# chpio/crdt-enc

Measured on AMD Instinct MI355X. Metric: op files compacted/sec + AEAD-open GB/s, 1M×4KiB ops/4096 actors, 1–8 GPUs, higher is better.
Workload: dtype u32; 1 GPU; C2: 1,048,576 x 4 KiB encrypted GCounter op files per GPU (4096 actors x 256 versions at N=1), decrypt + max-join + compact; plaintext_bytes=4085, actors=4096, parallelism=single GPU

## Files before the change

crdt-enc_amd/crdtenc.py:

```python
import ctypes
import os

HERE = os.path.dirname(os.path.abspath(__file__))
LIB_PATH = os.environ.get("CRDTENC_LIB") or os.path.join(HERE, "libcrdtenc.so")

OK = 0
STATUS_NAMES = {
    0: "OK", 1: "OUTER_LEN", 2: "OUTER_VERSION", 3: "KEY_VERSION", 4: "KEY_LEN",
    5: "PARSE_VBOX", 6: "DATA_VERSION", 7: "PARSE_ENCBOX", 8: "NONCE_LEN", 9: "AUTH",
    10: "PT_LEN", 11: "PT_VERSION", 12: "DECODE", 13: "OP_VERSION", 64: "INVALID_ARG",
    65: "DEVICE", 66: "NO_KEY", 67: "IO", 68: "NO_LOCAL_META", 69: "SHARD",
}
ERR_OP_VERSION, ERR_SHARD = 13, 69
SHARD_BAD, SHARD_GAP, SHARD_E0_MISMATCH = 1, 2, 4
STATE_VCLOCK, STATE_GCOUNTER, STATE_ORSWOT, STATE_MVREG, STATE_PNCOUNTER = 0, 1, 2, 3, 4
STATE_GSET = 5
OPEN_CREATE, COMPACT_INGEST_FORMAT, OPEN_MULTI_KEY = 1, 2, 4

CORE_VERSION = bytes.fromhex("e834d789101b463498239de990a9051f")
KEY_VERSION = bytes.fromhex("5df28591439a4cef8ca68433276cc9ed")

EXPORTS = [
    "ce_buf_free", "ce_status_str", "ce_ctx_create", "ce_ctx_destroy", "ce_ctx_set_stream",
    "ce_ctx_synchronize", "ce_ctx_last_error", "ce_cryptor_gen_key", "ce_cryptor_encrypt",
    "ce_cryptor_decrypt", "ce_cryptor_sealed_len", "ce_cryptor_decrypt_batch",
    "ce_cryptor_encrypt_batch", "ce_cryptor_decrypt_batch_device",
    "ce_cryptor_encrypt_batch_device", "ce_storage_open", "ce_storage_close",
    "ce_storage_list_op_actors", "ce_storage_load_ops", "ce_storage_store_ops",
    "ce_storage_remove_ops", "ce_storage_list_state_names", "ce_storage_store_state",
    "ce_storage_load_state", "ce_storage_remove_state", "ce_content_name", "ce_content_name_async",
    "ce_content_name_wait", "ce_core_open",
    "ce_core_close", "ce_core_set_latest_key", "ce_core_info_actor", "ce_core_read_remote",
    "ce_core_compact", "ce_core_apply_ops", "ce_core_state_bytes", "ce_core_ingest_ops",
    "ce_core_ingest_ops_device", "ce_core_ingest_states", "ce_core_compact_to_buffer",
    "ce_core_compact_into", "ce_core_compact_ops_device",
    "ce_core_register_actors", "ce_core_dense_capacity", "ce_core_export_dense",
    "ce_core_import_dense", "ce_vbuf_init", "ce_vbuf_remaining", "ce_vbuf_chunk",
    "ce_vbuf_advance", "ce_vbuf_chunks_vectored", "ce_ctx_set_timing", "ce_ctx_timing_read",
    "ce_ctx_timing_reset", "ce_ctx_set_timing_only", "ce_core_reset", "ce_core_settle", "ce_core_merge_state", "ce_core_dense_ready",
    "ce_keys_decode", "ce_keys_from_remote_metas", "ce_keys_merge", "ce_keys_free",
    "ce_keys_count", "ce_keys_latest", "ce_keys_get", "ce_keys_at", "ce_core_set_keys",
    "ce_core_apply_ops_batch", "ce_core_ingest_ops_iov", "ce_core_ingest_states_iov", "ce_core_compact_ops_iov",
    "ce_core_path_count", "ce_ctx_clock_probe",
    "ce_shard_owner", "ce_shard_owners", "ce_shard_stats_len", "ce_core_shard_stats",
    "ce_core_shard_window", "ce_core_ingest_ops_device_sharded", "ce_core_pending_export",
    "ce_core_pending_commit", "ce_core_writer_versions", "ce_shard_stats_host",
    "ce_shard_window_host", "ce_shard_window_exact", "ce_core_compact_ops_device_into",
    "ce_core_state_bytes_device", "ce_core_merge_state_device", "ce_core_export_columns_device",
    "ce_core_merge_columns_device", "ce_core_ingest_states_device",
    "ce_core_compact_into_async", "ce_core_compact_wait", "ce_host_alloc", "ce_host_free", "ce_content_names",
    "ce_core_gset_ingest_ops_device_sharded", "ce_core_gset_pending_members", "ce_core_gset_pending_commit",
    "ce_core_set_contains_device", "ce_core_set_contains", "ce_core_set_len", "ce_core_set_members_device",
    "ce_core_counter_read", "ce_core_clock_get", "ce_core_read_clock", "ce_core_orswot_member_clocks",
    "ce_core_mvreg_read",
]


class _HostMem:

    def __init__(self, n):
        self.p = lib().ce_host_alloc(n)
        if not self.p:
            raise MemoryError("ce_host_alloc(%d)" % n)

    def __del__(self):
        try:
# ... 285 lines not shown

    def set_timing(self, enable=True):
        self.check(lib().ce_ctx_set_timing(self.p, 1 if enable else 0), "set_timing")

    def set_timing_only(self, kernel=None):
        self.check(lib().ce_ctx_set_timing_only(self.p, kernel.encode() if kernel else None),
                   "set_timing_only")

    def timing(self, kernel):
        ms = ctypes.c_double(0)
        cnt = ctypes.c_uint64(0)
        self.check(lib().ce_ctx_timing_read(self.p, kernel.encode(), ctypes.byref(ms),
                                            ctypes.byref(cnt)), "timing")
        return ms.value, cnt.value

    def timing_reset(self):
        lib().ce_ctx_timing_reset(self.p)

    def clock_probe(self, out_ptr, blocks, samples, ticks, stream_ptr=None):
        self.check(lib().ce_ctx_clock_probe(self.p, ctypes.c_void_p(stream_ptr), ctypes.c_void_p(out_ptr),
                                            ctypes.c_uint32(blocks), ctypes.c_uint32(samples),
                                            ctypes.c_uint32(ticks)), "clock_probe")

    def gen_key(self):
        b = Buf()
        self.check(lib().ce_cryptor_gen_key(self.p, ctypes.byref(b)), "gen_key")
        vb = _take(b)
        return vb[:16], vb[16:]

    def encrypt(self, key, clear, nonce=None, key_version=KEY_VERSION):
        b = Buf()
        rc = lib().ce_cryptor_encrypt(self.p, _cbuf(key_version), _cbuf(key),
                                      ctypes.c_size_t(len(key)),
                                      _cbuf(nonce) if nonce is not None else None,
                                      _cbuf(clear), ctypes.c_size_t(len(clear)), ctypes.byref(b))
        self.check(rc, "encrypt")
        return _take(b)

    def decrypt(self, key, enc, key_version=KEY_VERSION):
        b = Buf()
        rc = lib().ce_cryptor_decrypt(self.p, _cbuf(key_version), _cbuf(key),
                                      ctypes.c_size_t(len(key)), _cbuf(enc),
                                      ctypes.c_size_t(len(enc)), ctypes.byref(b))
        if rc:
            return rc, None
        return 0, _take(b)
# ... 599 lines not shown
```

crdt-enc_amd/csrc/ce_core.cpp:

```cpp
#include <algorithm>
#include <atomic>
#include <cstdio>
#include <functional>
#include <set>

#include "ce_core.h"
#include "ce_shard.h"

using namespace ce;

namespace ce {


bool skip_any(Rd& r, int depth) {
  if (depth > 1024) return false;
  uint64_t at, cnt = 0;
  if (r.i >= r.n) return false;
  const uint8_t m = r.p[r.i];
  bool cont = false;
  if ((m & 0xf0) == 0x80) { r.i++; cnt = 2ull * (m & 15); cont = true; }
  else if ((m & 0xf0) == 0x90) { r.i++; cnt = m & 15; cont = true; }
  else if (m == 0xdc || m == 0xdd || m == 0xde || m == 0xdf) {
    r.i++;
    if (!rd_be(r, (m == 0xdc || m == 0xde) ? 2 : 4, &cnt)) return false;
// ... 784 lines not shown
    if (rg) return rg;
  }
  DecodeArgs da{};
  da.pt = ctx->out.as<uint8_t>();
  da.blob = d_blob;
  da.params = ctx->params.as<FileParams>();
  da.aux = ctx->poly_aux.as<PolyAux>();
  da.status = ctx->status.as<int32_t>();
  da.n = n;
  da.supported = c->d_supported.as<uint8_t>();
  da.n_supported = (uint32_t)c->supported.size();
  da.apply = ctx->apply.as<uint8_t>();
  da.counters = ctx->counters.as<uint32_t>();
  da.miss_list = ctx->miss.as<uint4>();
  da.miss_cap = 65536;
  da.refold = ctx->refold.as<uint8_t>();
  da.table = c->d_table.as<ActorSlot>();
  da.mask = c->cap - 1;
  da.nil_actor = table_has_nil(c);
  da.batch = c->d_batch.as<unsigned long long>();
  da.large_list = ctx->large.as<uint32_t>();

  ctx->open_log.grid_cap = test_grid_cap();
  auto run_fold = [&](const uint8_t* only) -> int {
    da.only = only;
    da.large_only = 1;
    if (pnc) {
      hipEvent_t t0, t1;
      (void)ctx->tlaunch("open_fold_small", &t0, &t1);
      if ((e = launch_open_fold_pn(ctx->stream, da, ctx->open_log, t0, t1))) return ctx->hip_fail(e, "fused");
    } else if (c->fused == 2 && c->files_per_wave != 1) {
      hipEvent_t t0, t1;
      (void)ctx->tlaunch("open_fold_small", &t0, &t1);
      if ((e = launch_open_fold_v2(ctx->stream, da, c->files_per_wave, ctx->open_log, t0, t1))) return ctx->hip_fail(e, "fused");
    } else {
      const int t = ctx->tbegin("open_fold_small");
      if ((e = launch_open_fold_small(ctx->stream, da, c->files_per_wave, ctx->open_log))) return ctx->hip_fail(e, "fused");
      ctx->tend(t);
    }
    count_open_launches(c, ctx);
    if (!setup_known) {
      if (hsetup_dev) {
        volatile const uint32_t* hp = hsetup;
        for (uint64_t i = 0; hp[16] != gen; i++) {
          if (i >= 64) sched_yield();
          if (i == (1ull << 22)) {
            if ((e = hipStreamSynchronize(ctx->stream))) return ctx->hip_fail(e, "setup counters");
          } else if (i > (1ull << 22) && hp[16] != gen) {
            return ctx->fail(CE_ERR_DEVICE, "setup counters never published");
// ... 1560 lines not shown
```

crdt-enc_amd/csrc/ce_ctx.cpp:

```cpp
#include <sys/random.h>

#include <algorithm>
#include <cstdio>

#include "ce_internal.h"

namespace ce {

hipError_t DevBuf::reserve(size_t bytes) {
  if (bytes <= cap) return hipSuccess;
  if (p) (void)hipFree(p);
  p = nullptr;
  cap = 0;
  size_t want = std::max<size_t>(bytes, 256);
  want = (want + 4095) & ~size_t(4095);
  hipError_t e = hipMalloc(&p, want);
  if (e == hipSuccess) cap = want;
  return e;
}
DevBuf::~DevBuf() {
  if (p) (void)hipFree(p);
}
hipError_t HostBuf::reserve(size_t bytes) {
  if (bytes <= cap) return hipSuccess;
// ... 14 lines not shown
  size_t got = 0;
  while (got < n) {
    ssize_t r = getrandom(out + got, n - got, 0);
    if (r > 0) got += (size_t)r;
  }
}

int32_t key_status(const KeyRef& k) {
  if (std::memcmp(k.version, kKeyVersion, 16) != 0) return CE_ERR_KEY_VERSION;
  if (k.len != 32) return CE_ERR_KEY_LEN;
  return CE_OK;
}

DevKey dev_key(const KeyRef& k) {
  DevKey d{};
  if (k.len == 32) std::memcpy(d.k, k.key, 32);
  return d;
}

uint32_t test_grid_cap() {
  const char* e = getenv("CE_TEST_GRID_CAP");
  const long v = e ? atol(e) : 0;
  return v < 1 ? 0u : (uint32_t)std::min<long>(v, 1l << 30);
}

uint32_t grid_waves_for(uint32_t work) {
  uint32_t full = 256u * 32u;
  if (const uint32_t cap = test_grid_cap()) full = std::min(full, cap);
  return std::max<uint32_t>(1, std::min<uint32_t>(work, full));
}

static int reserve_batch(ce_ctx* ctx, uint32_t n, uint64_t blob_len, uint32_t* extra_cap,
                         uint32_t seg_blocks = kSegBlocks) {
  const uint64_t ec = blob_len / (seg_blocks * 16) + 16;
  if (ec > 0xffffffffull) return ctx->fail(CE_ERR_INVALID_ARG, "batch too large");
  *extra_cap = (uint32_t)ec;
  hipError_t e;
  if ((e = ctx->params.reserve((size_t)n * sizeof(FileParams))) != hipSuccess ||
      (e = ctx->status.reserve((size_t)n * 4 + 64)) != hipSuccess ||
      (e = ctx->counters.reserve(256)) != hipSuccess ||
      (e = ctx->extra.reserve(ec * 8)) != hipSuccess ||
      (e = ctx->multi.reserve(ec * 4)) != hipSuccess ||
      (e = ctx->partials.reserve(ec * 2 * 5 * 4)) != hipSuccess ||
      (e = ctx->large.reserve((size_t)n * 4 + 64)) != hipSuccess ||
      (e = ctx->h_counters.reserve(256)) != hipSuccess)
    return ctx->hip_fail(e, "reserve batch scratch");
// ... 45 lines not shown
}

int device_open(ce_ctx* ctx, const uint8_t* d_blob, const uint64_t* d_offs, uint32_t n,
                uint64_t blob_len, bool outer, const KeyRef& key, uint8_t* d_out,
                int32_t* d_status, bool sync_counters, bool small_lanes, const DecodeArgs* ds) {
  uint32_t ec;
  int rc = reserve_batch(ctx, n, blob_len, &ec);
  if (rc) return rc;
  hipError_t e;
  if ((e = reset_counters(ctx)) != hipSuccess) return ctx->hip_fail(e, "memset counters");
  SegScratch sc = segscratch(ctx, ec);
  FileParams* P = ctx->params.as<FileParams>();
  static const bool ds8_on = !(getenv("CE_DS8") && atoi(getenv("CE_DS8")) == 0);
  const bool want_aux = small_lanes && ds && ds->ds.on && ds->ds.big && ds8_on;
  if (want_aux && (e = ctx->poly_aux.reserve((size_t)n * sizeof(PolyAux))) != hipSuccess)
    return ctx->hip_fail(e, "reserve poly aux");
  int t = ctx->tbegin("open_setup");
  if ((e = launch_open_setup(ctx->stream, d_blob, d_offs, n, outer, dev_key(key), key_status(key),
                             P, d_status, sc, want_aux ? ctx->poly_aux.as<PolyAux>() : nullptr)) != hipSuccess)
    return ctx->hip_fail(e, "open setup");
  ctx->tend(t);
  if (small_lanes) {
    ctx->open_log.grid_cap = test_grid_cap();
    DecodeArgs da{};
    da.pt = d_out;
    da.blob = d_blob;
    da.params = P;
    da.status = d_status;
    da.n = n;
    da.counters = ctx->counters.as<uint32_t>();
    if (ds) {
      da.ds = ds->ds;
      da.aux = want_aux ? ctx->poly_aux.as<PolyAux>() : nullptr;
      da.supported = ds->supported;
      da.n_supported = ds->n_supported;
      da.table = ds->table;
      da.mask = ds->mask;
    }
    t = ctx->tbegin("open_small");
    if ((e = launch_open_small_v2(ctx->stream, da, ctx->open_log)) != hipSuccess) return ctx->hip_fail(e, "open small");
    ctx->tend(t);
  }
  t = ctx->tbegin("segments_open");
  if ((e = launch_segments(ctx->stream, false, d_blob, d_out, P, n, d_status, sc,
                           grid_waves_for(n + ec), small_lanes)) != hipSuccess)
    return ctx->hip_fail(e, "open segments");
// ... 203 lines not shown
  return CE_OK;
}

int ce_ctx_set_timing_only(ce_ctx* c, const char* kernel) {
  if (!c) return CE_ERR_INVALID_ARG;
  std::lock_guard<std::recursive_mutex> g(c->mu);
  c->timing_only = kernel ? kernel : "";
  return CE_OK;
}

int ce_ctx_clock_probe(ce_ctx* c, void* hip_stream, uint64_t* d_out, uint32_t blocks,
                       uint32_t samples, uint32_t ticks) {
  if (!c || !d_out || blocks == 0 || blocks > 4096 || samples == 0 || ticks == 0 ||
      (uint64_t)samples * ticks > 100000000ull)
    return CE_ERR_INVALID_ARG;
  std::lock_guard<std::recursive_mutex> g(c->mu);
  (void)hipSetDevice(c->device);
  const hipError_t e = launch_clock_probe(hip_stream ? (hipStream_t)hip_stream : c->stream,
                                          reinterpret_cast<unsigned long long*>(d_out), blocks,
                                          samples, ticks);
  return e == hipSuccess ? CE_OK : c->hip_fail(e, "clock probe");
}

int ce_ctx_timing_read(ce_ctx* c, const char* kernel, double* total_ms, uint64_t* launches) {
  if (!c || !kernel || !total_ms || !launches) return CE_ERR_INVALID_ARG;
  std::lock_guard<std::recursive_mutex> g(c->mu);
  (void)hipStreamSynchronize(c->stream);
  double tot = 0;
  uint64_t cnt = 0;
  for (auto& t : c->timed) {
    if (std::strcmp(t.name, kernel) != 0) continue;
    float ms = 0;
    if (hipEventElapsedTime(&ms, t.a, t.b) == hipSuccess) { tot += ms; cnt++; }
  }
  *total_ms = tot;
  *launches = cnt;
  return CE_OK;
}

void ce_ctx_timing_reset(ce_ctx* c) {
  if (!c) return;
  std::lock_guard<std::recursive_mutex> g(c->mu);
  (void)hipStreamSynchronize(c->stream);
  for (auto& t : c->timed) { c->event_pool.push_back(t.a); c->event_pool.push_back(t.b); }
  c->timed.clear();
}
// ... 175 lines not shown
```

crdt-enc_amd/csrc/ce_fused.hip:

```cpp
#include <algorithm>

#include <hip/hip_ext.h>

#include "ce_device.h"
#include "ce_gset_device.h"

namespace ce {

static constexpr uint32_t kRegion = 64 * kKsStride - 16;

#ifndef CE_NCH
#define CE_NCH 2
#endif
template <int LPF>
struct FusedCfg {
  static constexpr int F = 64 / LPF;
  static constexpr int WPB = LPF == 16 ? 2 : 4;
  static constexpr int LOG = LPF == 16 ? 4 : LPF == 32 ? 5 : 6;
  static constexpr int WAVES_PER_SIMD = LPF == 16 ? 2 : LPF == 32 ? 3 : 4;
  static constexpr int NCH = LPF * CE_NCH <= 64 ? CE_NCH : 64 / LPF;
  static constexpr int LOGCH = NCH == 4 ? 2 : NCH == 2 ? 1 : 0;
};

template <int CTRL>
// ... 1323 lines not shown
        gs_put(G->committed, G->batch, v);
      }
      remaining -= todo;
    }
  }
  if (live && st != CE_OK && sub == 0) {
    a.status[f] = st;
    atomicAdd(&a.counters[3], 1u);
    atomicMin(&a.counters[5], f);
  }
}

__device__ const uint32_t kPolyOne[8] = {1u, 0u, 0u, 0u, 0u, 0u, 0u, 0u};

template <bool PAIR, bool EARLY, bool PN = false, bool GS = false>
__global__ __launch_bounds__(64, 2)
void k_open_fold_v3(DecodeArgs a) {
  constexpr int LPF = 16, F = 4, BPL = 4;
  __shared__ __attribute__((aligned(16))) uint8_t lds[(F - 1) * kRegionStride2 + kRegion2 + 64];
  const uint32_t lane = threadIdx.x & 63;
  const uint32_t grp = lane / LPF, sub = lane % LPF;
  uint8_t* fl = lds + grp * kRegionStride2;
  const uint32_t ngroups = (a.n + F - 1) / F;
  const uint32_t g_end = (uint32_t)(((uint64_t)(blockIdx.x + 1) * ngroups) / gridDim.x);
  uint32_t g = bcast((uint32_t)(((uint64_t)blockIdx.x * ngroups) / gridDim.x));
  FilePre2 nx = load_pre2(a, g * F + grp);
  const SupVers sup(a);
  DecState S{PN ? 51u : 38u, 0, 0, 0, 0, 0xffffffffu};
  GsCounts gsc;
  AuthFails fails;
  const uint32_t qpos = (sub + 15u) & 15u;
  const uint32_t qx = qpos & 3u, qy = qpos >> 2;
  static_assert(offsetof(FileParams, rpow) == 80, "rpow offset");
  auto wsrc = [&](uint32_t q, uint32_t aux_off, uint32_t rp_idx, const uint8_t*& base, uint32_t& stride) {
    base = q == 0 ? reinterpret_cast<const uint8_t*>(kPolyOne)
         : q == 3 ? reinterpret_cast<const uint8_t*>(a.aux) + aux_off
                  : reinterpret_cast<const uint8_t*>(a.params) + 80u + 20u * rp_idx;
    stride = q == 0 ? 0u : q == 3 ? (uint32_t)sizeof(PolyAux) : (uint32_t)sizeof(FileParams);
  };
  const uint8_t* x_base;
  const uint8_t* y_base;
  uint32_t x_stride, y_stride;
  wsrc(qx, (uint32_t)offsetof(PolyAux, r12), qx + 1u, x_base, x_stride);
  wsrc(qy, (uint32_t)offsetof(PolyAux, r48), qy + 3u, y_base, y_stride);

  uint4 ct[BPL][4];
  for (; g < g_end; g++) {
    const uint32_t f = g * F + grp;
    const FilePre2 cur = nx;
    if (EARLY) nx = load_pre2(a, (g + 1) * F + grp);
    const bool act = cur.ok && cur.len <= kSmallMax;
    const uint32_t len = act ? cur.len : 0u;
    const uint32_t npc = (len + 15) >> 4;
    const int32_t nblk = (int32_t)((len + 63) >> 6);
    const FileParams* Pp = a.params + (act ? f : 0);
    const PolyAux* Xp = a.aux + (act ? f : 0);
    const uint8_t* src = act ? a.blob + (((uint64_t)cur.in_hi << 32) | cur.in_off)
                             : reinterpret_cast<const uint8_t*>(a.params);
#pragma unroll
    for (int k = BPL - 1; k >= 0; k--) {
      const int32_t b = nblk - 1 - (int32_t)sub - LPF * k;
      if (k > 0) {
        const uint8_t* bp = b >= 0 ? src + 64u * (uint32_t)b : reinterpret_cast<const uint8_t*>(a.params);
#pragma unroll
        for (int j = 0; j < 4; j++) ct[k][j] = *reinterpret_cast<const uint4*>(bp + 16 * j);
      } else {
#pragma unroll
        for (int j = 0; j < 4; j++) {
          const uint32_t q = (uint32_t)(4 * b + j);
          const uint32_t off = b >= 0 ? 16u * (q < npc ? q : npc - 1u) : 0u;
          ct[0][j] = *reinterpret_cast<const uint4*>(src + off);
        }
      }
// ... 97 lines not shown
    }

    L5 v = mulmod(mulmod(acc, X), Y);
#pragma unroll
    for (int k = 0; k < 4; k++) {
#pragma unroll
      for (int i = 0; i < 5; i++) v.v[i] += row_down(v.v[i], 1 << k);
    }
    uint64_t d[5] = {LR.v[0], LR.v[1], LR.v[2], LR.v[3], LR.v[4]};
    mac5(d, v, mul_r(E6));
    mac5(d, glast, mul_r(R2));
    const L5 tot = reduce5(d);
    bool tag_ok = false;
    if (act && sub == 0) {
      tag_ok = poly_check(tot, ts);
      if (!tag_ok) a.status[f] = CE_ERR_AUTH;
    }
    fails.add(act && sub == 0 && !tag_ok, f);
    const bool ok = grp_bits<LPF>(tag_ok, grp) != 0;

    if (CE_V3_PRIO) __builtin_amdgcn_s_setprio(CE_V3_PRIO);
    if constexpr (GS) {
      decode_gset_lds<LPF>(a, sup, fl, len, act && ok, cur.apply != 0, f, grp, sub, gsc, [&] {
        if (!EARLY) nx = load_pre2(a, (g + 1) * F + grp);
      });
    } else {
      decode_fold<LPF, true, PN>(a, sup, fl, len, act && ok, cur.apply != 0, f, grp, sub, S, [&] {
        if (!EARLY) nx = load_pre2(a, (g + 1) * F + grp);
      });
    }
    if (CE_V3_PRIO) __builtin_amdgcn_s_setprio(0);
    __builtin_amdgcn_wave_barrier();
  }
  if constexpr (GS) gsc.flush(a);
  else flush_pending<LPF>(a, sub, S.pslot, S.pbest);
  fails.flush(a);
}

template <bool PF>
__global__ __launch_bounds__(64, 2)
void k_open_ds8(DecodeArgs a) {
  constexpr int LPF = 8, F = 8, BPL = 4;
  constexpr uint32_t kStride = kDsFuseRegion + 64;
  __shared__ __attribute__((aligned(16))) uint8_t lds[F * kStride + F * kDsAuxHalves * 2];
  const uint32_t lane = threadIdx.x & 63;
  const uint32_t grp = lane / LPF, sub = lane % LPF;
  uint8_t* fl = lds + grp * kStride;
  uint16_t* aux = reinterpret_cast<uint16_t*>(lds + F * kStride) + grp * kDsAuxHalves;
  const uint32_t ngroups = (a.n + F - 1) / F;
  const uint32_t g_end = (uint32_t)(((uint64_t)(blockIdx.x + 1) * ngroups) / gridDim.x);
  uint32_t g = bcast((uint32_t)(((uint64_t)blockIdx.x * ngroups) / gridDim.x));
  FilePre2 nx = load_pre2(a, g * F + grp);
  const SupVers sup(a);
  AuthFails fails;
  const uint32_t qpos = (sub + 7u) & 7u;
  const uint32_t qx = qpos & 3u;
  const bool x_one = qx == 0, y_one = (qpos >> 2) == 0, x_aux = qx == 3;
  const uint32_t x_off = x_aux ? (uint32_t)offsetof(PolyAux, r12) : 80u + 20u * (qx + 1u);
  uint4 ct[BPL][4];
// ... 188 lines not shown
      hipLaunchKernelGGL(k_open_ds8<true>, grid, dim3(64), 0, s, a);
    } else {
      static const uint32_t res = resident_blocks(k_open_ds8<false>, 64);
      const dim3 grid(log.grid(std::min<uint32_t>((a.n + 7) / 8, res), "open_ds8_nopf"));
      hipLaunchKernelGGL(k_open_ds8<false>, grid, dim3(64), 0, s, a);
    }
    DecodeArgs b = a;
    b.only = a.ds.big;
    launch_v2<16, 3, false, false, true>(s, b, log, "open_ds16");
  } else if (a.ds.on) {
    launch_v2<16, 3, false, false, true>(s, a, log, "open_ds16");
  } else {
    launch_v2<16, 3, false, false>(s, a, log, "open_only_lpf16");
  }
  return hipGetLastError();
}

hipError_t launch_open_fold_pn(hipStream_t s, const DecodeArgs& a, OpenLaunchLog& log, hipEvent_t t0,
                               hipEvent_t t1) {
  if (a.n == 0) return hipSuccess;
  if (!a.aux) return hipErrorInvalidValue;
  static const uint32_t res = resident_blocks(k_open_fold_v3<false, true, true>, 64);
  const dim3 grid(log.grid(std::min<uint32_t>((a.n + 3) / 4, res), "open_v3_pn"));
  if (t0) hipExtLaunchKernelGGL((k_open_fold_v3<false, true, true>), grid, dim3(64), 0, s, t0, t1, 0u, a);
  else hipLaunchKernelGGL((k_open_fold_v3<false, true, true>), grid, dim3(64), 0, s, a);
  return hipGetLastError();
}

hipError_t launch_open_fold_gset(hipStream_t s, const DecodeArgs& a, OpenLaunchLog& log, hipEvent_t t0,
                                 hipEvent_t t1) {
  if (a.n == 0) return hipSuccess;
  if (!a.aux || !a.gs) return hipErrorInvalidValue;
  static const uint32_t res = resident_blocks(k_open_fold_v3<false, true, false, true>, 64);
  const dim3 grid(log.grid(std::min<uint32_t>((a.n + 3) / 4, res), "open_v3_gset"));
  if (t0) hipExtLaunchKernelGGL((k_open_fold_v3<false, true, false, true>), grid, dim3(64), 0, s, t0, t1, 0u, a);
  else hipLaunchKernelGGL((k_open_fold_v3<false, true, false, true>), grid, dim3(64), 0, s, a);
  return hipGetLastError();
}

hipError_t launch_open_fold_v2(hipStream_t s, const DecodeArgs& a, int files_per_wave, OpenLaunchLog& log,
                               hipEvent_t t0, hipEvent_t t1) {
  if (a.n == 0) return hipSuccess;
  static const bool force_v2 = getenv("CE_FUSED_V2") != nullptr;
  if (files_per_wave == 4 && a.aux && !force_v2) {
    static const int v3 = [] {
      const char* e = getenv("CE_V3");
      return e ? atoi(e) : 2;
    }();
    auto go = [&](auto kern, const char* key) {
      const uint32_t res = resident_blocks(kern, 64);
      const dim3 grid(log.grid(std::min<uint32_t>((a.n + 3) / 4, res), key));
      if (t0) hipExtLaunchKernelGGL(kern, grid, dim3(64), 0, s, t0, t1, 0u, a);
      else hipLaunchKernelGGL(kern, grid, dim3(64), 0, s, a);
    };
    switch (v3 & 3) {
      case 1: go(k_open_fold_v3<true, false>, "open_v3_p1e0"); break;
      case 2: go(k_open_fold_v3<false, true>, "open_v3_p0e1"); break;
      case 3: go(k_open_fold_v3<true, true>, "open_v3_p1e1"); break;
      default: go(k_open_fold_v3<false, false>, "open_v3_p0e0"); break;
    }
    return hipGetLastError();
  }
  if (files_per_wave == 2) launch_v2<32, 3, true>(s, a, log, "open_v2_lpf32", t0, t1);
  else launch_v2<16, 2, false>(s, a, log, "open_v2_lpf16", t0, t1);
  return hipGetLastError();
}

__global__ void k_gate_runs(GateArgs g) {
  const uint32_t i = blockIdx.x * blockDim.x + threadIdx.x;
  if (i >= g.n) return;
  const uint32_t a = g.fa[i];
  if (a >= g.m) { atomicOr(&g.flags[0], 1u); return; }
  if (i == 0 || g.fa[i - 1] != a) {
    if (atomicAdd(&g.run_count[a], 1u) != 0) atomicOr(&g.flags[0], 1u);
    g.run_first[a] = i;
    if (g.fv[i] > g.e0[a]) atomicMin(&g.flags[1], i);
// ... 34 lines not shown
```

crdt-enc_amd/csrc/ce_gset_host.cpp:

```cpp
#include <algorithm>
#include <cstring>

#include "ce_core.h"
#include "ce_dotset.h"
#include "ce_dotset_io.h"
#include "ce_gset.h"
#include "ce_shard.h"

namespace ce {

struct GsState {
  DevBuf slots, bslots;
  DevBuf meta;
  uint32_t cap = 0, bcap = 0;
  bool batch_dirty = false;
  DevBuf col, sorted, vals, sort_tmp, scan_tmp, only;
  DevBuf gate;
  DevBuf fused;
  GsFused h_fused;
  DevBuf rd;
  HostBuf h_rd;
  uint64_t head_hint = 1u << 14;
};

// ... 677 lines not shown
  hipError_t e;
  int rc;
  uint32_t ec = 0;
  if ((rc = device_open_setup(ctx, d_blob, d_offs, n, blob_len, true, key_of(c), ctx->status.as<int32_t>(), &ec)))
    return rc;
  uint32_t* paths = g->meta.as<uint32_t>() + 12;
  g->h_fused = GsFused{committed(g), batch(g), paths};
  if ((e = g->fused.reserve(sizeof(GsFused))) || (e = hipMemsetAsync(paths, 0, 12, ctx->stream)) ||
      (e = hipMemcpyAsync(g->fused.p, &g->h_fused, sizeof(GsFused), hipMemcpyHostToDevice, ctx->stream)))
    return ctx->hip_fail(e, "gset fused args");
  DecodeArgs da{};
  da.pt = ctx->out.as<uint8_t>();
  da.blob = d_blob;
  da.params = ctx->params.as<FileParams>();
  da.status = ctx->status.as<int32_t>();
  da.n = n;
  da.supported = c->d_supported.as<uint8_t>();
  da.n_supported = (uint32_t)c->supported.size();
  da.apply = ctx->apply.as<uint8_t>();
  da.counters = ctx->counters.as<uint32_t>();
  da.aux = ctx->poly_aux.as<PolyAux>();
  da.gs = g->fused.as<GsFused>();
  ctx->open_log.grid_cap = test_grid_cap();
  {
    hipEvent_t t0, t1;
    (void)ctx->tlaunch("open_fold_small", &t0, &t1);
    if ((e = launch_open_fold_gset(ctx->stream, da, ctx->open_log, t0, t1))) return ctx->hip_fail(e, "fused");
  }
  g->batch_dirty = true;
  const SegScratch sc = segscratch(ctx, ec);
  int t = ctx->tbegin("segments_open");
  if ((e = launch_segments(ctx->stream, false, d_blob, ctx->out.as<uint8_t>(), ctx->params.as<FileParams>(), n,
                           ctx->status.as<int32_t>(), sc, grid_waves_for(n + ec), true)))
    return ctx->hip_fail(e, "open segments");
  ctx->tend(t);
  t = ctx->tbegin("finalize_open");
  if ((e = launch_finalize_multi(ctx->stream, false, ctx->out.as<uint8_t>(), ctx->params.as<FileParams>(),
                                 ctx->status.as<int32_t>(), sc, n)))
    return ctx->hip_fail(e, "open finalize");
  ctx->tend(t);
  count_open_launches(c, ctx);
  uint32_t hm[kMetaWords], hc[16];
  if ((e = hipMemcpyAsync(hc, ctx->counters.p, 64, hipMemcpyDeviceToHost, ctx->stream))) return ctx->hip_fail(e, "counters");
  if ((rc = read_meta(c, hm))) return rc;
  std::vector<int32_t> st;
  if (hm[4 + kGsOverflow]) {
// ... 221 lines not shown
```

crdt-enc_amd/csrc/ce_internal.h:

```cpp
#pragma once
#include <utility>
#include <hip/hip_runtime.h>
#include <hsa/hsa.h>
#include <sched.h>

#include <array>
#include <cstring>
#include <mutex>
#include <string>
#include <unordered_map>
#include <functional>
#include <vector>

#include "ce_common.h"
#include "ce_kernels.h"
#include "crdtenc.h"

namespace ce {

using Uuid = std::array<uint8_t, 16>;

struct UuidHash {
  size_t operator()(const Uuid& u) const {
    uint32_t w[4];
// ... 90 lines not shown
  uint32_t auth_failed = 0;
  uint32_t first_fail = 0xffffffffu;
};

}

namespace ce {
struct Uploader;
struct HostPool;
}

struct ce_storage {
  std::string local, remote;
};

struct ce_ctx {
  int device = 0;
  hipStream_t stream = nullptr;
  bool own_stream = false;
  std::recursive_mutex mu;
  std::string last_error;
  ce::DevBuf params, status, counters, extra, multi, partials, large, out, apply, refold, miss,
      supported, blob, offs, nonces, out_offs, outer_ver, batch_counters, split, segrec, redo, heads,
      poly_aux;
  ce::OpenLaunchLog open_log;
  ce::HostBuf h_counters, h_apply, h_stage, h_stage2, h_heads;
  uint32_t publish_gen = 0;
  hipEvent_t setup_ev = nullptr;
  hipStream_t side = nullptr;
  hipEvent_t side_ev = nullptr;
  hipEvent_t up_ev = nullptr;
  ce::Uploader* up = nullptr;
  ce::HostPool* pool = nullptr;
  bool timing = false;
  struct TimedLaunch {
    const char* name;
    hipEvent_t a, b;
  };
  std::vector<TimedLaunch> timed;
  std::vector<hipEvent_t> event_pool;
  hipEvent_t take_event() {
    if (!event_pool.empty()) {
      hipEvent_t e = event_pool.back();
      event_pool.pop_back();
      return e;
    }
    hipEvent_t e = nullptr;
// ... 49 lines not shown
DevKey dev_key(const KeyRef& k);

int device_open_setup(ce_ctx* ctx, const uint8_t* d_blob, const uint64_t* d_offs, uint32_t n,
                      uint64_t blob_len, bool outer, const KeyRef& key, int32_t* d_status,
                      uint32_t* extra_cap, FillArgs* fills = nullptr,
                      const std::function<int()>* after_fill = nullptr);
SegScratch segscratch(ce_ctx* ctx, uint32_t extra_cap);
int device_open(ce_ctx* ctx, const uint8_t* d_blob, const uint64_t* d_offs, uint32_t n,
                uint64_t blob_len, bool outer, const KeyRef& key, uint8_t* d_out,
                int32_t* d_status, bool sync_counters, bool small_lanes = false,
                const DecodeArgs* ds = nullptr);

int device_seal(ce_ctx* ctx, const uint8_t* d_clear, const uint64_t* d_offs, uint32_t n,
                uint64_t clear_len_total, const uint8_t* d_outer_version, const uint8_t* d_nonces,
                uint8_t* d_out, const uint64_t* d_out_offs, const KeyRef& key, bool counters_ready = false);
uint32_t* ctx_counters(ce_ctx* ctx);

int seal_one(ce_ctx* ctx, const KeyRef& key, const uint8_t* outer_version, const uint8_t* nonce,
             const uint8_t* clear, size_t clear_len, std::vector<uint8_t>* file,
             const uint8_t* prefix16 = nullptr);

uint32_t grid_waves_for(uint32_t work);
uint32_t test_grid_cap();

struct DmaD2H {
  bool ok = false;
  hsa_agent_t gpu{0}, cpu{0};
  uint32_t engine = 0;
};
bool dma_init(int device, DmaD2H* out);
bool dma_d2h(const DmaD2H& d, void* dst, const void* src, size_t n, hsa_signal_t sig);
void dma_wait(hsa_signal_t sig);
bool dma_signal(hsa_signal_t* sig);
void dma_signal_destroy(hsa_signal_t sig);

int stage_host_batch(ce_ctx* ctx, const uint8_t* const* files, const uint64_t* offs, uint32_t n);
void destroy_uploader(ce_ctx* ctx);
void host_parallel_for(ce_ctx* ctx, uint32_t n, const std::function<void(uint32_t)>& fn);

}
```

crdt-enc_amd/csrc/ce_kernels.h:

```cpp
#pragma once
#include <hip/hip_runtime.h>
#include <stdint.h>

#include "ce_common.h"

namespace ce {

static constexpr uint32_t kPageBytes = 4096;
static constexpr uint32_t kSegPages = 4;
static constexpr uint32_t kSegBlocks = kSegPages * kPageBytes / 16;
static constexpr uint32_t kSmallMax = kPageBytes;

struct alignas(16) FileParams {
  uint32_t subkey[8];
  uint32_t n2[2];
  uint32_t pad0[2];
  uint32_t s[4];
  uint32_t tag[4];
  uint32_t rpow[7][5];
  uint32_t pad1;
  uint64_t in_off;
  uint64_t out_off;
  uint32_t len;
  int32_t status;
// ... 80 lines not shown
  int32_t* status;
  uint32_t n;
  const uint8_t* supported;
  uint32_t n_supported;
  const uint8_t* apply;
  const ActorSlot* table;
  uint32_t mask;
  unsigned long long* batch;
  uint32_t* counters;
  union {
    uint4* miss_list;
    const struct GsFused* gs;
  };
  uint32_t miss_cap;
  uint8_t* refold;
  const uint8_t* only;
  int large_only;
  const uint32_t* large_list;
  const uint8_t* blob;
  uint8_t* redo;
  int nil_actor;
  DsFuse ds;
  const PolyAux* aux;
};
hipError_t launch_decode_dots(hipStream_t s, const DecodeArgs& a, uint32_t grid_waves);
hipError_t launch_decode_pn_ops(hipStream_t s, const DecodeArgs& a, uint32_t grid_waves);
hipError_t launch_clock_probe(hipStream_t s, unsigned long long* out, uint32_t blocks,
                              uint32_t samples, uint32_t ticks);

static constexpr uint32_t kSplitParts = 16;
static constexpr uint32_t kSplitMinDots = 2048;
static constexpr uint32_t kSplitDone = 0xfffffffeu;
struct SplitScratch {
  uint4* part;
};
hipError_t launch_decode_split(hipStream_t s, const DecodeArgs& a, SplitScratch sp, uint32_t n_large);
hipError_t launch_segments_decode(hipStream_t s, const uint8_t* in, uint8_t* out, const DecodeArgs& da,
                                  SegScratch sc, uint32_t grid_waves, uint4* rec);
hipError_t launch_segdec_apply(hipStream_t s, const DecodeArgs& a, SegScratch sc, const uint4* rec,
                               uint32_t n_large);

struct OpenLaunchLog {
  uint32_t grid_cap = 0;
  uint32_t n = 0;
  const char* took[8];
  void note(const char* key) {
    if (n < 8) took[n++] = key;
  }
  uint32_t grid(uint32_t blocks, const char* key) {
    note(key);
    if (grid_cap == 0 || blocks <= grid_cap) return blocks;
    note("open_grid_capped");
    return grid_cap;
  }
};

hipError_t launch_open_fold_small(hipStream_t s, const DecodeArgs& a, int files_per_wave, OpenLaunchLog& log);
hipError_t launch_open_fold_v2(hipStream_t s, const DecodeArgs& a, int files_per_wave, OpenLaunchLog& log,
                               hipEvent_t t0 = nullptr, hipEvent_t t1 = nullptr);
hipError_t launch_open_fold_pn(hipStream_t s, const DecodeArgs& a, OpenLaunchLog& log,
                               hipEvent_t t0 = nullptr, hipEvent_t t1 = nullptr);
hipError_t launch_open_fold_gset(hipStream_t s, const DecodeArgs& a, OpenLaunchLog& log,
                                 hipEvent_t t0 = nullptr, hipEvent_t t1 = nullptr);
hipError_t launch_open_small_v2(hipStream_t s, const DecodeArgs& a, OpenLaunchLog& log);

struct GateArgs {
  const uint32_t* fa;
  const uint64_t* fv;
  uint32_t n, m;
  const uint64_t* e0;
  uint32_t* run_count;
  uint32_t* run_first;
  uint32_t* flags;
  unsigned long long* newnov;
  uint8_t* apply;
  unsigned long long* newnov_host;
// ... 46 lines not shown
```

crdt-enc_amd/csrc/ce_kernels.hip:

```cpp
#include "ce_device.h"

namespace ce {

__global__ __launch_bounds__(256) void k_open_setup(const uint8_t* __restrict__ blob,
                                                    const uint64_t* __restrict__ offs, uint32_t n,
                                                    int outer, DevKey key, int32_t key_status,
                                                    FileParams* __restrict__ params,
                                                    int32_t* __restrict__ status, SegScratch sc,
                                                    PolyAux* __restrict__ aux) {
  __shared__ uint4 stage[256 * 8];
  const uint32_t f = blockIdx.x * blockDim.x + threadIdx.x;
  const bool active = f < n;
  const uint64_t off = active ? offs[f] : 0;
  const uint64_t flen = active ? offs[f + 1] - off : 0;
  const uint8_t* enc = blob + off;
  uint64_t enc_len = flen;
  int32_t st = active ? CE_OK : CE_ERR_OUTER_LEN;
  if (active && outer) {
    if (flen < 16) st = CE_ERR_OUTER_LEN;
    else {
      const uint4 v = *reinterpret_cast<const uint4*>(enc);
      auto le = [](int i) {
        return (uint32_t)kCoreVersion[4 * i] | ((uint32_t)kCoreVersion[4 * i + 1] << 8) |
               ((uint32_t)kCoreVersion[4 * i + 2] << 16) | ((uint32_t)kCoreVersion[4 * i + 3] << 24);
// ... 1187 lines not shown
    if (ln) put(nov_at + tpn + (at & 0xffff), a, vn);
    if (ls) put(st_at + tps + (at >> 16), a, vs);
    if constexpr (PN) {
      const uint32_t atq = block_scan_1024(lq, ws, &tot);
      if (lq) put(q_at + tpq + atq, a, vq);
    }
  }
}

hipError_t launch_open_setup(hipStream_t s, const uint8_t* blob, const uint64_t* offs, uint32_t n,
                             bool outer, DevKey key, int32_t key_status, FileParams* params,
                             int32_t* status, SegScratch sc, PolyAux* aux) {
  if (n == 0) return hipSuccess;
  hipLaunchKernelGGL(k_open_setup, dim3((n + 255) / 256), dim3(256), 0, s, blob, offs, n,
                     outer ? 1 : 0, key, key_status, params, status, sc, aux);
  return hipGetLastError();
}

__global__ void k_fill(FillArgs a) {
  const uint32_t r = blockIdx.y;
  if ((int)r == a.n) {
    if (blockIdx.x == 0 && threadIdx.x < 16)
      a.counters[threadIdx.x] = (threadIdx.x == 5 || threadIdx.x == 13) ? 0xffffffffu : 0u;
    return;
  }
  const FillRange f = a.r[r];
  const uint64_t t0 = blockIdx.x * (uint64_t)blockDim.x + threadIdx.x, ts = (uint64_t)gridDim.x * blockDim.x;
  const uint64_t head = ((16 - (reinterpret_cast<uintptr_t>(f.p) & 15)) & 15) / 4;
  const bool vec = (reinterpret_cast<uintptr_t>(f.p) & 3) == 0 &&
                   (!f.src || ((reinterpret_cast<uintptr_t>(f.src) ^ reinterpret_cast<uintptr_t>(f.p)) & 15) == 0) &&
                   f.words > head + 4;
  if (!vec) {
    for (uint64_t i = t0; i < f.words; i += ts) f.p[i] = f.src ? f.src[i] : f.value;
    return;
  }
  const uint64_t body = (f.words - head) / 4, tail0 = head + 4 * body;
  uint4* p4 = reinterpret_cast<uint4*>(f.p + head);
  if (f.src) {
    const uint4* s4 = reinterpret_cast<const uint4*>(f.src + head);
    for (uint64_t i = t0; i < body; i += ts) p4[i] = s4[i];
  } else {
    const uint4 v = make_uint4(f.value, f.value, f.value, f.value);
    for (uint64_t i = t0; i < body; i += ts) p4[i] = v;
  }
  if (t0 < head) f.p[t0] = f.src ? f.src[t0] : f.value;
  if (t0 < f.words - tail0) f.p[tail0 + t0] = f.src ? f.src[tail0 + t0] : f.value;
// ... 356 lines not shown
```

include/crdtenc.h:

```cpp
#ifndef CRDTENC_H
#define CRDTENC_H

#include <stddef.h>
#include <stdint.h>

#ifdef __cplusplus
extern "C" {
#endif

enum ce_status {
  CE_OK = 0,
  CE_ERR_OUTER_LEN = 1,
  CE_ERR_OUTER_VERSION = 2,
  CE_ERR_KEY_VERSION = 3,
  CE_ERR_KEY_LEN = 4,
  CE_ERR_PARSE_VBOX = 5,
  CE_ERR_DATA_VERSION = 6,
  CE_ERR_PARSE_ENCBOX = 7,
  CE_ERR_NONCE_LEN = 8,
  CE_ERR_AUTH = 9,
  CE_ERR_PT_LEN = 10,
  CE_ERR_PT_VERSION = 11,
  CE_ERR_DECODE = 12,
  CE_ERR_OP_VERSION = 13,
// ... 6 lines not shown
};

typedef struct ce_buf {
  uint8_t *data;
  size_t len;
} ce_buf;

void ce_buf_free(ce_buf *b);
const char *ce_status_str(int status);

typedef struct ce_ctx ce_ctx;

int ce_ctx_create(int device, ce_ctx **out);
void ce_ctx_destroy(ce_ctx *ctx);
int ce_ctx_set_stream(ce_ctx *ctx, void *hip_stream);
void ce_ctx_synchronize(ce_ctx *ctx);
const char *ce_ctx_last_error(ce_ctx *ctx);
int ce_ctx_set_timing(ce_ctx *ctx, int enable);
int ce_ctx_set_timing_only(ce_ctx *ctx, const char *kernel);
int ce_ctx_timing_read(ce_ctx *ctx, const char *kernel, double *total_ms, uint64_t *launches);
void ce_ctx_timing_reset(ce_ctx *ctx);
int ce_ctx_clock_probe(ce_ctx *ctx, void *hip_stream, uint64_t *d_out, uint32_t blocks,
                       uint32_t samples, uint32_t ticks);

int ce_cryptor_gen_key(ce_ctx *ctx, ce_buf *out);

int ce_cryptor_encrypt(ce_ctx *ctx, const uint8_t key_version[16], const uint8_t *key,
                       size_t key_len, const uint8_t *nonce, const uint8_t *clear,
                       size_t clear_len, ce_buf *out);

int ce_cryptor_decrypt(ce_ctx *ctx, const uint8_t key_version[16], const uint8_t *key,
                       size_t key_len, const uint8_t *enc, size_t enc_len, ce_buf *out);

size_t ce_cryptor_sealed_len(size_t clear_len);

int ce_cryptor_decrypt_batch(ce_ctx *ctx, const uint8_t key_version[16], const uint8_t *key,
                             size_t key_len, const uint8_t *blob, const uint64_t *offs,
                             uint32_t n, uint8_t *out_blob, uint64_t *out_offs,
                             uint64_t *out_lens, int32_t *status);

int ce_cryptor_encrypt_batch(ce_ctx *ctx, const uint8_t key_version[16], const uint8_t *key,
                             size_t key_len, const uint8_t *blob, const uint64_t *offs,
                             uint32_t n, const uint8_t *nonces, uint8_t *out_blob,
                             size_t out_cap, uint64_t *out_offs);

int ce_cryptor_decrypt_batch_device(ce_ctx *ctx, const uint8_t key_version[16],
// ... 197 lines not shown
```

Before: 358.8 million op files/s.

## Add hybrid static/dynamic work-stealing schedule to open_fold_v3 kernel

Replaces the even static split of file groups across blocks in k_open_fold_v3 with a hybrid schedule. Each block first takes a fixed share (half by default), then draws chunks of 4 groups from a global atomic ticket counter, which is reset before each launch. This is meant to cut tail imbalance when some waves run slower than others. It costs one atomic per chunk and a memset per fold, and adds optional per-wave timestamp instrumentation behind an env var.

```diff
diff --git a/crdt-enc_amd/crdtenc.py b/crdt-enc_amd/crdtenc.py
--- a/crdt-enc_amd/crdtenc.py
+++ b/crdt-enc_amd/crdtenc.py
@@ -41,7 +41,7 @@
     "ce_keys_decode", "ce_keys_from_remote_metas", "ce_keys_merge", "ce_keys_free",
     "ce_keys_count", "ce_keys_latest", "ce_keys_get", "ce_keys_at", "ce_core_set_keys",
     "ce_core_apply_ops_batch", "ce_core_ingest_ops_iov", "ce_core_ingest_states_iov", "ce_core_compact_ops_iov",
-    "ce_core_path_count", "ce_ctx_clock_probe",
+    "ce_core_path_count", "ce_ctx_clock_probe", "ce_ctx_wave_stamps",
     "ce_shard_owner", "ce_shard_owners", "ce_shard_stats_len", "ce_core_shard_stats",
     "ce_core_shard_window", "ce_core_ingest_ops_device_sharded", "ce_core_pending_export",
     "ce_core_pending_commit", "ce_core_writer_versions", "ce_shard_stats_host",
@@ -373,6 +373,16 @@
                                             ctypes.c_uint32(blocks), ctypes.c_uint32(samples),
                                             ctypes.c_uint32(ticks)), "clock_probe")
 
+    def wave_stamps(self):
+        import numpy as np
+        n = ctypes.c_uint32(0)
+        self.check(lib().ce_ctx_wave_stamps(self.p, None, ctypes.c_uint32(0), ctypes.byref(n)), "wave_stamps")
+        out = np.zeros((n.value, 4), dtype=np.uint64)
+        if n.value:
+            self.check(lib().ce_ctx_wave_stamps(self.p, ctypes.c_void_p(out.ctypes.data), ctypes.c_uint32(n.value),
+                                                ctypes.byref(n)), "wave_stamps")
+        return out[:n.value]
+
     def gen_key(self):
         b = Buf()
         self.check(lib().ce_cryptor_gen_key(self.p, ctypes.byref(b)), "gen_key")
diff --git a/crdt-enc_amd/csrc/ce_core.cpp b/crdt-enc_amd/csrc/ce_core.cpp
--- a/crdt-enc_amd/csrc/ce_core.cpp
+++ b/crdt-enc_amd/csrc/ce_core.cpp
@@ -830,9 +830,13 @@
   da.large_list = ctx->large.as<uint32_t>();
 
   ctx->open_log.grid_cap = test_grid_cap();
+  ctx->open_log.stamps = test_wave_stamps(ctx);
+  ctx->open_log.stamp_waves = 0;
   auto run_fold = [&](const uint8_t* only) -> int {
     da.only = only;
     da.large_only = 1;
+    if (only && (e = hipMemsetAsync(ctx->counters.as<uint32_t>() + kTicketWord, 0, 4, ctx->stream)))
+      return ctx->hip_fail(e, "ticket");
     if (pnc) {
       hipEvent_t t0, t1;
       (void)ctx->tlaunch("open_fold_small", &t0, &t1);
diff --git a/crdt-enc_amd/csrc/ce_ctx.cpp b/crdt-enc_amd/csrc/ce_ctx.cpp
--- a/crdt-enc_amd/csrc/ce_ctx.cpp
+++ b/crdt-enc_amd/csrc/ce_ctx.cpp
@@ -60,6 +60,17 @@
   const char* e = getenv("CE_TEST_GRID_CAP");
   const long v = e ? atol(e) : 0;
   return v < 1 ? 0u : (uint32_t)std::min<long>(v, 1l << 30);
+}
+
+unsigned long long* test_wave_stamps(ce_ctx* ctx) {
+  const char* e = getenv("CE_TEST_WAVE_STAMPS");
+  if (!e || atoi(e) < 1) return nullptr;
+  const size_t bytes = (size_t)kStampWaves * kStampWords * 8;
+  if (ctx->stamps.reserve(bytes) != hipSuccess || hipMemsetAsync(ctx->stamps.p, 0, bytes, ctx->stream) != hipSuccess) {
+    (void)hipGetLastError();
+    return nullptr;
+  }
+  return ctx->stamps.as<unsigned long long>();
 }
 
 uint32_t grid_waves_for(uint32_t work) {
@@ -151,6 +162,8 @@
   ctx->tend(t);
   if (small_lanes) {
     ctx->open_log.grid_cap = test_grid_cap();
+    ctx->open_log.stamps = nullptr;
+    ctx->open_log.stamp_waves = 0;
     DecodeArgs da{};
     da.pt = d_out;
     da.blob = d_blob;
@@ -400,6 +413,22 @@
   return e == hipSuccess ? CE_OK : c->hip_fail(e, "clock probe");
 }
 
+int ce_ctx_wave_stamps(ce_ctx* c, uint64_t* out, uint32_t cap_waves, uint32_t* n_waves) {
+  if (!c || !n_waves || (cap_waves && !out)) return CE_ERR_INVALID_ARG;
+  std::lock_guard<std::recursive_mutex> g(c->mu);
+  (void)hipSetDevice(c->device);
+  const uint32_t n = c->stamps.p ? c->open_log.stamp_waves : 0;
+  *n_waves = n;
+  const uint32_t k = std::min(n, cap_waves);
+  if (k == 0) return CE_OK;
+  hipError_t e;
+  if ((e = hipMemcpyAsync(out, c->stamps.p, (size_t)k * kStampWords * 8, hipMemcpyDeviceToHost, c->stream)) ||
+      (e = hipStreamSynchronize(c->stream)))
+    return c->hip_fail(e, "wave stamps");
+  for (uint32_t i = 0; i < k; i++) out[(size_t)kStampWords * i + 3] = (uint64_t)CE_DYN_CHUNK | ((uint64_t)CE_DYN_STATIC_PCT << 32);
+  return CE_OK;
+}
+
 int ce_ctx_timing_read(ce_ctx* c, const char* kernel, double* total_ms, uint64_t* launches) {
   if (!c || !kernel || !total_ms || !launches) return CE_ERR_INVALID_ARG;
   std::lock_guard<std::recursive_mutex> g(c->mu);
diff --git a/crdt-enc_amd/csrc/ce_fused.hip b/crdt-enc_amd/csrc/ce_fused.hip
--- a/crdt-enc_amd/csrc/ce_fused.hip
+++ b/crdt-enc_amd/csrc/ce_fused.hip
@@ -1369,9 +1369,25 @@
   const uint32_t grp = lane / LPF, sub = lane % LPF;
   uint8_t* fl = lds + grp * kRegionStride2;
   const uint32_t ngroups = (a.n + F - 1) / F;
-  const uint32_t g_end = (uint32_t)(((uint64_t)(blockIdx.x + 1) * ngroups) / gridDim.x);
-  uint32_t g = bcast((uint32_t)(((uint64_t)blockIdx.x * ngroups) / gridDim.x));
-  FilePre2 nx = load_pre2(a, g * F + grp);
+  const uint32_t fixed = (uint32_t)((uint64_t)(ngroups / gridDim.x) * CE_DYN_STATIC_PCT / 100u);
+  const uint32_t dyn0 = fixed * gridDim.x;
+  uint32_t tk = 0;
+  auto draw = [&] {
+    uint32_t tw = kTicketWord;
+    asm volatile("" : "+v"(tw));
+    if (lane == 0) tk = atomicAdd(a.counters + tw, 1u);
+  };
+  auto chunk = [&](uint32_t& lo, uint32_t& hi) {
+    const uint64_t s = dyn0 + (uint64_t)bcast(tk) * CE_DYN_CHUNK;
+    lo = s < ngroups ? (uint32_t)s : ngroups;
+    hi = ngroups - lo < CE_DYN_CHUNK ? ngroups : lo + CE_DYN_CHUNK;
+    draw();
+  };
+  draw();
+  uint32_t gn = bcast(blockIdx.x * fixed), c_end = gn + fixed;
+  if (fixed == 0) chunk(gn, c_end);
+  if (a.stamps && lane == 0) a.stamps[(uint64_t)kStampWords * blockIdx.x] = __builtin_amdgcn_s_memrealtime();
+  FilePre2 nx = load_pre2(a, gn * F + grp);
   const SupVers sup(a);
   DecState S{PN ? 51u : 38u, 0, 0, 0, 0, 0xffffffffu};
   GsCounts gsc;
@@ -1392,10 +1408,11 @@
   wsrc(qy, (uint32_t)offsetof(PolyAux, r48), qy + 3u, y_base, y_stride);
 
   uint4 ct[BPL][4];
-  for (; g < g_end; g++) {
-    const uint32_t f = g * F + grp;
+  while (gn < ngroups) {
+    const uint32_t f = gn * F + grp;
     const FilePre2 cur = nx;
-    if (EARLY) nx = load_pre2(a, (g + 1) * F + grp);
+    if (++gn == c_end) chunk(gn, c_end);
+    if (EARLY) nx = load_pre2(a, gn * F + grp);
     const bool act = cur.ok && cur.len <= kSmallMax;
     const uint32_t len = act ? cur.len : 0u;
     const uint32_t npc = (len + 15) >> 4;
@@ -1539,11 +1556,11 @@
     if (CE_V3_PRIO) __builtin_amdgcn_s_setprio(CE_V3_PRIO);
     if constexpr (GS) {
       decode_gset_lds<LPF>(a, sup, fl, len, act && ok, cur.apply != 0, f, grp, sub, gsc, [&] {
-        if (!EARLY) nx = load_pre2(a, (g + 1) * F + grp);
+        if (!EARLY) nx = load_pre2(a, gn * F + grp);
       });
     } else {
       decode_fold<LPF, true, PN>(a, sup, fl, len, act && ok, cur.apply != 0, f, grp, sub, S, [&] {
-        if (!EARLY) nx = load_pre2(a, (g + 1) * F + grp);
+        if (!EARLY) nx = load_pre2(a, gn * F + grp);
       });
     }
     if (CE_V3_PRIO) __builtin_amdgcn_s_setprio(0);
@@ -1552,6 +1569,16 @@
   if constexpr (GS) gsc.flush(a);
   else flush_pending<LPF>(a, sub, S.pslot, S.pbest);
   fails.flush(a);
+  if (a.stamps) {
+    const unsigned long long t_out = __builtin_amdgcn_s_memrealtime();
+    const unsigned long long hw = (uint32_t)__builtin_amdgcn_s_getreg((31 << 11) | 4) |
+                                  ((unsigned long long)(uint32_t)__builtin_amdgcn_s_getreg((3 << 11) | 20) << 32);
+    if (lane == 0) {
+      unsigned long long* o = a.stamps + (uint64_t)kStampWords * blockIdx.x;
+      o[1] = t_out;
+      o[2] = hw;
+    }
+  }
 }
 
 template <bool PF>
@@ -1786,8 +1813,9 @@
   if (!a.aux) return hipErrorInvalidValue;
   static const uint32_t res = resident_blocks(k_open_fold_v3<false, true, true>, 64);
   const dim3 grid(log.grid(std::min<uint32_t>((a.n + 3) / 4, res), "open_v3_pn"));
-  if (t0) hipExtLaunchKernelGGL((k_open_fold_v3<false, true, true>), grid, dim3(64), 0, s, t0, t1, 0u, a);
-  else hipLaunchKernelGGL((k_open_fold_v3<false, true, true>), grid, dim3(64), 0, s, a);
+  const DecodeArgs b = log.stamped(a, grid.x);
+  if (t0) hipExtLaunchKernelGGL((k_open_fold_v3<false, true, true>), grid, dim3(64), 0, s, t0, t1, 0u, b);
+  else hipLaunchKernelGGL((k_open_fold_v3<false, true, true>), grid, dim3(64), 0, s, b);
   return hipGetLastError();
 }
 
@@ -1797,8 +1825,9 @@
   if (!a.aux || !a.gs) return hipErrorInvalidValue;
   static const uint32_t res = resident_blocks(k_open_fold_v3<false, true, false, true>, 64);
   const dim3 grid(log.grid(std::min<uint32_t>((a.n + 3) / 4, res), "open_v3_gset"));
-  if (t0) hipExtLaunchKernelGGL((k_open_fold_v3<false, true, false, true>), grid, dim3(64), 0, s, t0, t1, 0u, a);
-  else hipLaunchKernelGGL((k_open_fold_v3<false, true, false, true>), grid, dim3(64), 0, s, a);
+  const DecodeArgs b = log.stamped(a, grid.x);
+  if (t0) hipExtLaunchKernelGGL((k_open_fold_v3<false, true, false, true>), grid, dim3(64), 0, s, t0, t1, 0u, b);
+  else hipLaunchKernelGGL((k_open_fold_v3<false, true, false, true>), grid, dim3(64), 0, s, b);
   return hipGetLastError();
 }
 
@@ -1814,8 +1843,9 @@
     auto go = [&](auto kern, const char* key) {
       const uint32_t res = resident_blocks(kern, 64);
       const dim3 grid(log.grid(std::min<uint32_t>((a.n + 3) / 4, res), key));
-      if (t0) hipExtLaunchKernelGGL(kern, grid, dim3(64), 0, s, t0, t1, 0u, a);
-      else hipLaunchKernelGGL(kern, grid, dim3(64), 0, s, a);
+      const DecodeArgs b = log.stamped(a, grid.x);
+      if (t0) hipExtLaunchKernelGGL(kern, grid, dim3(64), 0, s, t0, t1, 0u, b);
+      else hipLaunchKernelGGL(kern, grid, dim3(64), 0, s, b);
     };
     switch (v3 & 3) {
       case 1: go(k_open_fold_v3<true, false>, "open_v3_p1e0"); break;
diff --git a/crdt-enc_amd/csrc/ce_gset_host.cpp b/crdt-enc_amd/csrc/ce_gset_host.cpp
--- a/crdt-enc_amd/csrc/ce_gset_host.cpp
+++ b/crdt-enc_amd/csrc/ce_gset_host.cpp
@@ -723,6 +723,8 @@
   da.aux = ctx->poly_aux.as<PolyAux>();
   da.gs = g->fused.as<GsFused>();
   ctx->open_log.grid_cap = test_grid_cap();
+  ctx->open_log.stamps = test_wave_stamps(ctx);
+  ctx->open_log.stamp_waves = 0;
   {
     hipEvent_t t0, t1;
     (void)ctx->tlaunch("open_fold_small", &t0, &t1);
diff --git a/crdt-enc_amd/csrc/ce_internal.h b/crdt-enc_amd/csrc/ce_internal.h
--- a/crdt-enc_amd/csrc/ce_internal.h
+++ b/crdt-enc_amd/csrc/ce_internal.h
@@ -136,7 +136,8 @@
   std::string last_error;
   ce::DevBuf params, status, counters, extra, multi, partials, large, out, apply, refold, miss,
       supported, blob, offs, nonces, out_offs, outer_ver, batch_counters, split, segrec, redo, heads,
-      poly_aux;
+      poly_aux,
+      stamps;
   ce::OpenLaunchLog open_log;
   ce::HostBuf h_counters, h_apply, h_stage, h_stage2, h_heads;
   uint32_t publish_gen = 0;
@@ -232,6 +233,7 @@
 
 uint32_t grid_waves_for(uint32_t work);
 uint32_t test_grid_cap();
+unsigned long long* test_wave_stamps(ce_ctx* ctx);
 
 struct DmaD2H {
   bool ok = false;
diff --git a/crdt-enc_amd/csrc/ce_kernels.h b/crdt-enc_amd/csrc/ce_kernels.h
--- a/crdt-enc_amd/csrc/ce_kernels.h
+++ b/crdt-enc_amd/csrc/ce_kernels.h
@@ -126,7 +126,18 @@
   int nil_actor;
   DsFuse ds;
   const PolyAux* aux;
-};
+  unsigned long long* stamps;
+};
+static constexpr uint32_t kTicketWord = 32;
+#ifndef CE_DYN_CHUNK
+#define CE_DYN_CHUNK 4u
+#endif
+#ifndef CE_DYN_STATIC_PCT
+#define CE_DYN_STATIC_PCT 50u
+#endif
+static_assert(CE_DYN_CHUNK >= 1 && CE_DYN_CHUNK <= 64 && CE_DYN_STATIC_PCT <= 100, "k_open_fold_v3 schedule");
+static constexpr uint32_t kStampWords = 4;
+static constexpr uint32_t kStampWaves = 16384;
 hipError_t launch_decode_dots(hipStream_t s, const DecodeArgs& a, uint32_t grid_waves);
 hipError_t launch_decode_pn_ops(hipStream_t s, const DecodeArgs& a, uint32_t grid_waves);
 hipError_t launch_clock_probe(hipStream_t s, unsigned long long* out, uint32_t blocks,
@@ -156,6 +167,14 @@
     if (grid_cap == 0 || blocks <= grid_cap) return blocks;
     note("open_grid_capped");
     return grid_cap;
+  }
+  unsigned long long* stamps = nullptr;
+  uint32_t stamp_waves = 0;
+  DecodeArgs stamped(const DecodeArgs& a, uint32_t blocks) {
+    DecodeArgs b = a;
+    b.stamps = blocks <= kStampWaves ? stamps : nullptr;
+    stamp_waves = b.stamps ? blocks : 0;
+    return b;
   }
 };
 
diff --git a/crdt-enc_amd/csrc/ce_kernels.hip b/crdt-enc_amd/csrc/ce_kernels.hip
--- a/crdt-enc_amd/csrc/ce_kernels.hip
+++ b/crdt-enc_amd/csrc/ce_kernels.hip
@@ -1233,6 +1233,7 @@
   if ((int)r == a.n) {
     if (blockIdx.x == 0 && threadIdx.x < 16)
       a.counters[threadIdx.x] = (threadIdx.x == 5 || threadIdx.x == 13) ? 0xffffffffu : 0u;
+    if (blockIdx.x == 0 && threadIdx.x == kTicketWord) a.counters[kTicketWord] = 0u;
     return;
   }
   const FillRange f = a.r[r];
diff --git a/include/crdtenc.h b/include/crdtenc.h
--- a/include/crdtenc.h
+++ b/include/crdtenc.h
@@ -52,6 +52,7 @@
 void ce_ctx_timing_reset(ce_ctx *ctx);
 int ce_ctx_clock_probe(ce_ctx *ctx, void *hip_stream, uint64_t *d_out, uint32_t blocks,
                        uint32_t samples, uint32_t ticks);
+int ce_ctx_wave_stamps(ce_ctx *ctx, uint64_t *out, uint32_t cap_waves, uint32_t *n_waves);
 
 int ce_cryptor_gen_key(ce_ctx *ctx, ce_buf *out);
 
```

Result: faster. 382.3 million op files/s, median of 6 (+6.6%).
